# iyioon/NYPC-Yacht-Auction

Hardware: AMD Instinct MI355X
Metric: MCTS node-expansions/sec/GPU @4096 envs x100 sims; episodes/sec 1-8 GPU (higher is better)
Workload: dtype f32

## Files before the change

### nypc-yacht-auction_amd/csrc/yk_engine.hip

```cpp
#include <math.h>

#include <algorithm>
#include <vector>

#include "yk_api.h"
#include "yk_common.h"
#include "yk_engine_dev.h"
#include "yk_forced.h"
#include "yk_fpu.h"
#include "yk_net.h"

#define YK_MAX_GROUPS 8

using namespace yk;

namespace {


struct PwPlan {
    int nleaf, nop, root;
    uint16_t start[64], len[64];
    uint8_t a[64], b[64];
};
constexpr int pw_build(PwPlan& p, int start, int n) {
// ... 62 lines not shown
    int l = 0;
    for (int i = 0; i < p.nleaf; i++) l = p.len[i] > l ? p.len[i] : l;
    return l;
}
static_assert(NCOMB > pw_lmax(), "two category starts could share a leaf of the pairwise plan");
static_assert(PF_WCAP % 8 == 0 && PF_WCAP >= 16 && GAMES_PER_BLOCK * PF_WCAP * 4 <= 40 * 1024,
              "the prior window: whole float4 pairs, a slot per category, 16 waves per CU");
constexpr int PW_NLEAF = make_plan().nleaf;
constexpr int PW_SPLIT = make_plan().start[PW_NLEAF / 2];
static_assert(PW_SPLIT % 8 == 0 && PW_SPLIT <= PF_WCAP && ASIZE - PW_SPLIT <= PF_WCAP,
              "both halves of the pairwise tree fit the prior window, float4s aligned");
static_assert(PW_SPLIT > NBID && (PW_SPLIT - NBID) / NCOMB < NCAT, "the split lies inside a category's block");
constexpr int PW_SPLIT_CAT = (PW_SPLIT - NBID) / NCOMB, PW_SPLIT_COMB = (PW_SPLIT - NBID) % NCOMB;
constexpr int pw_leaf2() {
    const PwPlan p = make_plan();
    int i = 0;
    while (ASIZE - p.start[i] > PF_WCAP) i++;
    return i;
}
constexpr int PW_LEAF2 = pw_leaf2(), PW_BASE2 = make_plan().start[PW_LEAF2];
static_assert(PW_LEAF2 <= PW_NLEAF / 2 && PW_BASE2 % 8 == 0 && PW_BASE2 <= PW_SPLIT - (PW_SPLIT_COMB & 3),
              "the second piece holds the right half and the group the split cuts");

struct ValidQ {
    int mode;
    int n;
    uint32_t used;
    __device__ __forceinline__ bool operator()(int a) const {
        if (mode == 1) return a < NBID;
        if (mode != 0 || a < NBID) return false;
        const int base = a - NBID, cat = base / NCOMB, ci = base - cat * NCOMB;
        if ((used >> cat) & 1u) return false;
        if (n >= 10) return true;
        if (n == 5) return ci == 0;
        return c_tab.comb_max[ci] < n;
    }
};
__device__ __forceinline__ ValidQ valid_q(const YkS& s) {
    ValidQ q;
    const int round = s_round(s), phase = s_phase(s);
    const uint64_t wa = s_pw(s, 0, 0);
    q.n = __builtin_amdgcn_readfirstlane(wa_n(wa));
    q.used = __builtin_amdgcn_readfirstlane((uint32_t)wa_used(wa));
    q.mode = __builtin_amdgcn_readfirstlane((phase == 0 && round != 13) ? 1 : (phase == 1 && q.n >= 5) ? 0 : -1);
    return q;
}


__device__ __forceinline__ void wave_sync() {
    __builtin_amdgcn_fence(__ATOMIC_ACQ_REL, "workgroup");
    __builtin_amdgcn_wave_barrier();
}

__device__ __forceinline__ float wave_max(float v) {
    v = fmaxf(v, xlane<32>(v));
    v = fmaxf(v, xlane<16>(v));
    v = fmaxf(v, xlane<8>(v));
    v = fmaxf(v, xlane<4>(v));
    v = fmaxf(v, xlane<2>(v));
    return fmaxf(v, xlane<1>(v));
}
__device__ __forceinline__ float softmax_p(float x, float m, float lse) { return exp_acc(x - m - lse); }
__device__ __forceinline__ float wave_sumf(float v) {
    v += xlane<32>(v);
    v += xlane<16>(v);
    v += xlane<8>(v);
    v += xlane<4>(v);
    v += xlane<2>(v);
    return v + xlane<1>(v);
}
__device__ __forceinline__ int wave_min_i(int v) {
    v = min(v, xlane<32>(v));
    v = min(v, xlane<16>(v));
    v = min(v, xlane<8>(v));
    v = min(v, xlane<4>(v));
    v = min(v, xlane<2>(v));
    return min(v, xlane<1>(v));
}

struct PyV {
    double v;
    uint32_t t;
};
__device__ __forceinline__ PyV pv_update(PyV q, uint32_t n, PyV v) {
    PyV prod, sum, out;
    if (q.t == T_F32) prod = PyV{(double)((float)n * (float)q.v), T_F32};
    else prod = PyV{(double)n * q.v, q.t};
    if (prod.t == T_F32 || v.t == T_F32) sum = PyV{(double)((float)prod.v + (float)v.v), T_F32};
    else if (prod.t == T_F64 || v.t == T_F64) sum = PyV{prod.v + v.v, T_F64};
    else sum = PyV{prod.v + v.v, T_INT};
    if (sum.t == T_F32) out = PyV{(double)((float)sum.v / (float)(n + 1)), T_F32};
    else out = PyV{sum.v / (double)(n + 1), T_F64};
    return out;
}

__global__ void k_lut(float* sq, float* sqe) {
    const int i = blockIdx.x * blockDim.x + threadIdx.x;
    if (i >= LUT_N) return;
    sq[i] = (float)sqrt((double)i);
    sqe[i] = (float)sqrt((double)i + 1e-8);
}

__global__ void k_reset(EngDev d, int start_games, uint32_t env_base) {
    const int e = blockIdx.x * blockDim.x + threadIdx.x;
    if (e >= d.E) return;
    for (int t = e; t < d.T; t += d.E) {
        d.node_count[t] = d.node_count[d.T + t] = 0;
        d.edge_count[t] = d.edge_count[d.T + t] = 0;
        d.arena_top[t] = 0;
        d.gen[t] = 0;
        d.cur_round[t] = 0;
        d.root_c[2 * t] = make_uint4(0, 0, 0, 0);
        d.root_c[2 * t + 1] = make_uint4(0, 0, RV_OFF, 0);
    }
#pragma unroll
    for (int k = 0; k < GST; k++) d.gstats[(long)e * GST + k] = 0;
    if (!start_games) return;
    d.env_id[e] = env_base + (uint32_t)e;
    Stream rs{d.seed, d.env_id[e], 0};
    YkS s;
#pragma unroll
    for (int k = 0; k < 8; k++) s.w[k] = 0;
    s.w[0] = 1ull | NO_BIDS;
    new_round_rolls(s, rs);
    st_state(d.board + e, s);
    d.cur[e] = 1;
    d.ctr[e] = rs.ctr;
    d.done[e] = 0;
    d.nmoves[e] = 0;
    d.rec_voff[(long)e * (d.M + 1)] = 0;
}

__global__ __launch_bounds__(256) void k_move_begin(EngDev d, int move, int external_root) {
    const int lane = threadIdx.x & 63;
    const int e = d.e_lo + blockIdx.x * GAMES_PER_BLOCK + (threadIdx.x >> 6);
    if (e >= d.e_hi) return;
    const int t = tree_of(d, e);
    if (lane == 0) {
        d.root_c[2 * t] = make_uint4(0, 0, 0, 0);
        d.root_c[2 * t + 1] = make_uint4(0, 0, RV_OFF, 0);
    }
    if (!external_root) {
        if (d.done[e]) return;
        const YkS b = ld_state(d.board + e);
        const YkS r = canonical(b, d.cur[e]);
        const bool idle = d.arena && (d.cur[e] == d.seat[e] ? d.arena_agent : d.arena_opp) != YK_PLAYER_MCTS;
        if (lane == 0) {
            st_state(d.root + e, r);
            d.rec_ctr[((long)e * d.M + move) * 2] = d.ctr[e];
            d.idle[e] = idle ? 1 : 0;
        }
        if (idle) return;
    } else if (lane == 0) {
        d.idle[e] = 0;
    }
    const YkS r = ld_state(d.root + e);
    const int rr = s_round(r);
    const int cr = d.cur_round[t];
    if (rr == cr) return;
    if (rr < cr) {
        if (lane == 0) atomicOr(d.err, ERR_ROUND);
        return;
    }
    const int g = d.gen[t], h = g ^ 1;
    uint32_t* hx = d.hidx[h] + (long)t * d.HCAP;
    for (int i = lane; i < d.HCAP; i += 64) hx[i] = 0;
    const NodeRec* src = d.nodes[g] + (long)t * d.NCAP;
    NodeRec* dst = d.nodes[h] + (long)t * d.NCAP;
    const Edge* esrc = d.edges[g] + (long)t * d.ECAP;
// ... 126 lines not shown
        gathered += (uint64_t)nv;
        return -1;
    }
    if (FPU) {
        const int mine = bj;
        wave_argmax_step(best, bj);
        const uint64_t own = __ballot(mine == bj);
        wtag = own ? __builtin_amdgcn_readlane(btag, (int)__builtin_ctzll(own)) : 0u;
        const bool vis = bj != 0x7FFFFFFF;
        if (found && vis) {
            const float fq = fpu_value((int64_t)fpu_wave_sum((uint64_t)fw), fpu_wave_sum(fm), Ns, fr);
            fcnt = 1;
            if (fpu_unvisited_wins(fq, ub, uj, best, bj)) {
                fcnt = 3;
                best = ub;
                bj = uj;
                wtag = 0u;
            }
        } else if (found) {
            best = ub;
            bj = uj;
            wtag = 0u;
        }
        if (FORCED) fpick = best == INFINITY;
        scanned += (uint64_t)nv + (uint64_t)walked;
        gathered += (uint64_t)nv;
        return bj;
    }
    if (lane == 0 && found && (ub > best || (ub == best && uj < bj))) {
        best = ub;
        bj = uj;
        btag = 0;
    }
    const int mine = bj;
    wave_argmax_step(best, bj);
    if (FORCED) fpick = best == INFINITY;
    const uint64_t own = __ballot(mine == bj);
    wtag = own ? __builtin_amdgcn_readlane(btag, (int)__builtin_ctzll(own)) : 0u;
    scanned += (uint64_t)nv + (uint64_t)walked;
    gathered += (uint64_t)nv;
    return bj;
}

__device__ __forceinline__ void select_none(const EngDev& d, int e, int lane) {
    if (lane == 0) {
        d.leaf_flag[e] = 0;
        d.path_len[e] = 0;
        d.end_node[e] = 0;
    }
}

template <bool FORCED, bool FPU>
__device__ __forceinline__ void select_game(const EngDev& d, int e, int lane, int t, int g, const uint32_t* env_ids,
                                            uint64_t* ctr_arr, const ForcedDev& fd, const FpuDev& fp) {
    int fpick = 0;
    int fcnt = 0;
    int fpu_n = 0, fpu_u = 0;
    YkS s = ld_state(d.root + e);
    Stream rs{d.seed, env_ids[e], ctr_arr[e]};
    const NodeRec* nodes = d.nodes[g] + (long)t * d.NCAP;
    const Edge* edges = d.edges[g] + (long)t * d.ECAP;
    const float* Pbase = d.arenaP + (long)t * d.AE;
    const uint16_t* Sbase = d.arenaS + (long)t * d.AE;
    uint64_t* path = d.path + (long)e * MAXD;
    int depth = 0;
    uint64_t scanned = 0, gathered = 0;
    int ngl = 0;
    int leaf = 0;
    uint32_t end_id = 0;
    PyV res{0.0, T_INT};
    bool have = false;
    int nid = -1;
    NodeF f{};
    bool pre = false;
    int pre_bj = 0x7FFFFFFF;
    uint32_t pre_tag = 0;
    {
        const uint4 rc = d.root_c[2 * t], rc1 = d.root_c[2 * t + 1];
        const uint32_t rid = uni(rc.x);
        if (rid != 0) {
            have = true;
            nid = (int)rid - 1;
            f = ld_node(nodes + nid);
            f.p_off = rc.y;
            f.nvalid = rc.z;
            f.vinfo = (uint64_t)rc1.x | ((uint64_t)rc1.y << 32);
            f = uniform(f);
        }
        if (rid != 0 && uni(rc1.z) != RV_OFF) {
            const float sq = (float)sqrt((double)f.Ns), sqe = (float)sqrt((double)f.Ns + 1e-8);
            pre_bj = __builtin_amdgcn_readfirstlane(root_scan<FORCED, FPU>(
                d, t, lane, rc1.z, Pbase + rc.y, Sbase + rc.y, edges, (int)rc.z, (int)rc.w, (int)rc1.w, sq, sqe, pre_tag,
                scanned, gathered, f.Ns, fd.k, fpick, fp.r_root, fcnt));
            pre_tag = __builtin_amdgcn_readfirstlane(pre_tag);
            pre = pre_bj != -1;
            if (FORCED) fpick = pre ? __builtin_amdgcn_readfirstlane(fpick) : 0;
            if (FPU && pre) {
                fcnt = __builtin_amdgcn_readfirstlane(fcnt);
                fpu_n += fcnt & 1;
                fpu_u += fcnt >> 1;
            }
        }
    }
    while (true) {
        if (!have) {
            const double es = game_ended(s, 1);
            if (es != 0.0) {
                res = PyV{-es, T_F64};
                break;
            }
            const uint64_t hsh = index_hash(s);
            nid = __builtin_amdgcn_readfirstlane(lookup(d, g, t, s, hsh, f));
            f = uniform(f);
            if (nid < 0) {
                leaf = 1;
                if (lane == 0) {
                    st_state(d.leaf_state + e, s);
                    d.leaf_hash[e] = hsh;
                }
                break;
            }
            if (depth == 0 && lane == 0) {
                d.root_c[2 * t] = make_uint4((uint32_t)nid + 1, f.p_off, f.nvalid, 0);
                d.root_c[2 * t + 1] = make_uint4((uint32_t)f.vinfo, (uint32_t)(f.vinfo >> 32), RV_OFF, 0);
            }
        }
        const uint32_t p_off = f.p_off;
        const int V = (int)f.nvalid;
        const uint64_t vinfo = f.vinfo;
        if (V == 0) {
            res = PyV{0.0, T_INT};
            end_id = (uint32_t)nid + 1;
            break;
        }
        const uint32_t Ns = f.Ns;
        const float sq = (float)sqrt((double)Ns);
        const float sqe = (float)sqrt((double)Ns + 1e-8);
        const float* P = Pbase + p_off;
        const uint16_t* S = Sbase + p_off;
        int bj_out;
        uint32_t wtag;
        if (depth == 0 && pre) {
            bj_out = pre_bj;
            wtag = pre_tag;
        } else {
            float best = -INFINITY;
            int bj = 0x7FFFFFFF;
            uint32_t btag = 0;
            float bestx = -INFINITY;
            int bjx = 0x7FFFFFFF;
            int64_t fw = 0;
            uint64_t fm = 0;
            int Vs = V;
            if (d.node_summary && Ns == 0) {
                bj = (int)f.first_j;
                Vs = 0;
            }
            float4 p4 = make_float4(0.f, 0.f, 0.f, 0.f);
            ushort4 s4 = make_ushort4(0, 0, 0, 0);
            if (lane * 4 < Vs) {
                p4 = *reinterpret_cast<const float4*>(P + lane * 4);
                s4 = *reinterpret_cast<const ushort4*>(S + lane * 4);
            }
            for (int j0 = lane * 4; j0 < Vs; j0 += 256) {
                const float pv[4] = {p4.x, p4.y, p4.z, p4.w};
                const uint16_t sv[4] = {s4.x, s4.y, s4.z, s4.w};
                Edge ev[4];
#pragma unroll
                for (int t = 0; t < 4; t++)
                    if (j0 + t < Vs && sv[t]) {
                        ev[t] = edges[sv[t] - 1];
                        ngl++;
                    }
                if (j0 + 256 < Vs) {
                    p4 = *reinterpret_cast<const float4*>(P + j0 + 256);
                    s4 = *reinterpret_cast<const ushort4*>(S + j0 + 256);
                }
#pragma unroll
                for (int t = 0; t < 4; t++) {
                    const int j = j0 + t;
                    if (j < Vs) {
                        float u;
                        const float cp = d.c32 * pv[t];
                        if (sv[t]) {
                            u = (float)ev[t].Q + (cp * sq) / (float)(ev[t].N + 1);
                            if (FORCED && depth == 0 && forced_edge(ev[t].N, pv[t], Ns, fd.k)) u = INFINITY;
                        } else {
                            u = cp * sqe;
                        }
                        if (FPU) {
                            if (sv[t]) {
                                fw += fpu_w_term(ev[t].N, ev[t].Q);
                                fm += fpu_m_term(pv[t]);
                                if (u > best) {
                                    best = u;
                                    bj = j;
                                    btag = ev[t].tag;
                                }
                            } else if (u > bestx) {
                                bestx = u;
                                bjx = j;
                            }
                        } else if (u > best) {
                            best = u;
                            bj = j;
                            btag = sv[t] ? ev[t].tag : 0u;
                        }
                    }
                }
            }
            if (Vs) wave_argmax_step(best, bj);
            if (FPU && Vs) {
                wave_argmax_step(bestx, bjx);
                const bool vis = bj != 0x7FFFFFFF, unv = bjx != 0x7FFFFFFF;
                bool unv_won = unv;
                if (vis && unv) {
                    const float fq = fpu_value((int64_t)fpu_wave_sum((uint64_t)fw), fpu_wave_sum(fm), Ns, depth == 0 ? fp.r_root : fp.r);
                    unv_won = fpu_unvisited_wins(fq, bestx, bjx, best, bj);
                    fpu_n++;
                    fpu_u += unv_won;
                }
                if (unv_won) {
                    best = bestx;
                    bj = bjx;
                    btag = 0u;
                }
            }
            if (FORCED && depth == 0) fpick = best == INFINITY;
            scanned += (uint64_t)Vs;
            bj_out = bj;
            wtag = __builtin_amdgcn_readlane(btag, __builtin_amdgcn_readfirstlane((bj & 255) >> 2));
        }
        const int bj = bj_out;
        int j = bj;
        if (j == 0x7FFFFFFF) j = 0;
        if (depth >= MAXD) {
            if (lane == 0) atomicOr(d.err, ERR_DEPTH);
            res = PyV{0.0, T_INT};
            break;
        }
        const uint32_t child = uni(bj == 0x7FFFFFFF ? 0u : (wtag >> 2));
        if (child) {
            if (lane == 0) path[depth] = ((uint64_t)(p_off + (uint32_t)j) << 32) | (uint32_t)nid | PATH_DET;
            depth++;
            have = true;
            nid = (int)child - 1;
            f = uniform(ld_node(nodes + nid));
            s = ld_state(reinterpret_cast<const yk_state_t*>(nodes[nid].key));
            continue;
        }
        have = false;
        const VInfo vi = unpack_vinfo(vinfo, (uint32_t)V);
        const int a = compact_to_action(vi, j);
        int np = 1;
        const uint64_t ctr0 = rs.ctr;
        const int st = step_state<true>(s, 1, a, rs, np);
        const uint32_t det = rs.ctr == ctr0 ? PATH_DET : 0u;
        if (lane == 0) path[depth] = ((uint64_t)(p_off + (uint32_t)j) << 32) | (uint32_t)nid | det;
        depth++;
        if (st != YK_ST_OK) {
            if (lane == 0) atomicOr(d.err, ERR_STEP);
            res = PyV{0.0, T_INT};
            break;
        }
        s = canonical(s, np);
    }
    gathered += (uint64_t)xlane_sum(ngl);
    if (lane == 0) {
        d.leaf_flag[e] = (uint8_t)(leaf ? (t < d.E ? 1 : 2) : 0);
        d.path_len[e] = (uint8_t)depth;
        d.end_node[e] = end_id;
        d.res_v[e] = res.v;
        d.res_t[e] = res.t;
        ctr_arr[e] = rs.ctr;
        unsigned long long* gs = reinterpret_cast<unsigned long long*>(d.gstats + (long)e * GST);
        atomicAdd(gs + 1, (unsigned long long)scanned);
        atomicAdd(gs + 2, (unsigned long long)depth);
        atomicAdd(gs + 7, 1ull);
        if (FORCED) atomicAdd(gs + 12, (unsigned long long)fpick);
        if (FPU) {
            atomicAdd(gs + 14, (unsigned long long)fpu_u);
            atomicAdd(gs + 15, (unsigned long long)fpu_n);
        }
        atomicAdd(gs + 8, (unsigned long long)gathered);
    }
}

__device__ __forceinline__ ForcedDev forced_arg() { return ForcedDev{0.0, 0.0}; }
__device__ __forceinline__ const ForcedDev& forced_arg(const ForcedDev& fd) { return fd; }
__device__ __forceinline__ ForcedDev forced_arg(const FpuDev&) { return ForcedDev{0.0, 0.0}; }
__device__ __forceinline__ const ForcedDev& forced_arg(const ForcedDev& fd, const FpuDev&) { return fd; }
__device__ __forceinline__ FpuDev fpu_arg() { return FpuDev{0.0, 0.0}; }
__device__ __forceinline__ FpuDev fpu_arg(const ForcedDev&) { return FpuDev{0.0, 0.0}; }
__device__ __forceinline__ const FpuDev& fpu_arg(const FpuDev& fp) { return fp; }
__device__ __forceinline__ const FpuDev& fpu_arg(const ForcedDev&, const FpuDev& fp) { return fp; }
template <bool FORCED, bool FPU, class... FD>
__global__ __launch_bounds__(256) __attribute__((amdgpu_waves_per_eu(4))) void k_select(EngDev d, const uint32_t* env_ids, uint64_t* ctr_arr, FD... fd) {
    static_assert(sizeof...(FD) == (FORCED ? 1 : 0) + (FPU ? 1 : 0), "ForcedDev with FORCED, FpuDev with FPU, no further argument");
    const int lane = threadIdx.x & 63;
    const int e = __builtin_amdgcn_readfirstlane(d.e_lo + blockIdx.x * GAMES_PER_BLOCK + (threadIdx.x >> 6));
    if (e >= d.e_hi) return;
    if (d.done[e] || d.idle[e]) {
        select_none(d, e, lane);
        return;
    }
    const int t = __builtin_amdgcn_readfirstlane(tree_of(d, e));
    const int g = __builtin_amdgcn_readfirstlane((int)d.gen[t]);
    select_game<FORCED, FPU>(d, e, lane, t, g, env_ids, ctr_arr, forced_arg(fd...), fpu_arg(fd...));
}

__device__ __forceinline__ void expand_backup_game(const EngDev& d, int e, int lane, int t, int g);
template <bool FORCED, bool FPU, class... FD>
__global__ __launch_bounds__(256) __attribute__((amdgpu_waves_per_eu(YK_EXPAND_WPE))) void k_expand_backup(
    EngDev d, int do_select, const uint32_t* env_ids, uint64_t* ctr_arr, FD... fd) {
    static_assert(sizeof...(FD) == (FORCED ? 1 : 0) + (FPU ? 1 : 0), "ForcedDev with FORCED, FpuDev with FPU, no further argument");
    const int lane = threadIdx.x & 63;
    const int e = __builtin_amdgcn_readfirstlane(d.e_lo + blockIdx.x * GAMES_PER_BLOCK + (threadIdx.x >> 6));
    if (e >= d.e_hi) return;
    if (d.done[e]) return;
    const int t = __builtin_amdgcn_readfirstlane(tree_of(d, e));
    const int g = __builtin_amdgcn_readfirstlane((int)d.gen[t]);
    const bool idle = d.idle[e] != 0;
    expand_backup_game(d, e, lane, t, g);
    if (do_select) {
        if (idle) {
            select_none(d, e, lane);
            return;
        }
        wave_sync();
        select_game<FORCED, FPU>(d, e, lane, t, g, env_ids, ctr_arr, forced_arg(fd...), fpu_arg(fd...));
    }
}

__device__ __forceinline__ void expand_backup_game(const EngDev& d, int e, int lane, int t, int g) {
    PyV res{d.res_v[e], d.res_t[e]};
    uint32_t end_id = 0;
    if (d.leaf_flag[e]) {
        const YkS s = ld_state(d.leaf_state + e);
        const uint64_t ihsh = d.leaf_hash[e];
        const uint64_t hsh = d.prior == 1 ? key_hash(s) : 0ull;
        const VInfo vi = valid_info(s, 1);
        const ValidQ valid = valid_q(s);
        const int V = vi.V;
        const int leaf = lane >> 1, h = lane & 1;
        const int st = c_pw.start[leaf], nl = c_pw.len[leaf], G = nl >> 3, R = nl & 7;
        float4 q[PW_GMAX];
        float qt[PW_TMAX];
        float v, mx = 0.f, lse = 0.f;
        const int pidx = (int)d.gstats[(long)e * GST + 0];
        const bool rec = d.rec_pred && (e % d.rec_stride) == 0 && pidx < d.max_exp;
        const long rslot = rec ? (long)(e / d.rec_stride) * d.max_exp + pidx : 0;
        bool masked = false;
        __shared__ __attribute__((aligned(16))) float s_win[GAMES_PER_BLOCK][PF_WCAP];
        float* win = s_win[threadIdx.x >> 6];
        int fast = 0, wbase = 0, wlen = 0;
        if (d.prior_fast && V > 0) {
            if (valid.mode == 0 && valid.n == 5) {
                fast = 2;
                wlen = 16;
            } else {
                const int a0 = __builtin_amdgcn_readfirstlane(compact_to_action(vi, 0));
                const int a1 = __builtin_amdgcn_readfirstlane(compact_to_action(vi, V - 1));
                wbase = a0 & ~7;
                wlen = (a1 + 1 - wbase + 7) & ~7;
                fast = wlen <= PF_WCAP ? 1 : 0;
            }
        }
        const auto wslot = [&](int a) { return fast == 2 ? (a - NBID) / NCOMB : a - wbase; };
        if (d.prior == 0) {
            const float2 ml = d.mlse[e];
            mx = ml.x;
            lse = ml.y;
            if (d.fparts > 1) {
                float ms = ml.y;
                for (int p = 1; p < d.fparts; p++) {
                    const float2 q = d.mlse[(long)p * d.E + e];
                    const float mm = fmaxf(mx, q.x);
                    if (mm != -INFINITY) {
                        ms = ms * exp_acc(mx - mm) + q.y * exp_acc(q.x - mm);
                        mx = mm;
                    }
                }
                lse = logf(ms);
            }
            v = d.vpred[e];
        } else {
            v = hash_prior_v(hsh);
        }
        if (fast) {
            for (int i = 4 * lane; i < wlen; i += 256) *reinterpret_cast<float4*>(win + i) = make_float4(0.f, 0.f, 0.f, 0.f);
            wave_sync();
            const float* __restrict__ xr = d.logits + (long)e * PI_LD;
            for (int j0 = lane; j0 < V; j0 += 256) {
                float xa[4];
                int aa[4];
#pragma unroll
                for (int u = 0; u < 4; u++) {
                    const int j = j0 + 64 * u;
                    aa[u] = j < V ? compact_to_action(vi, j) : 0;
                    xa[u] = (d.prior == 0 && j < V) ? xr[aa[u]] : 0.f;
                }
#pragma unroll
                for (int u = 0; u < 4; u++)
                    if (j0 + 64 * u < V)
                        win[wslot(aa[u])] = d.prior == 0 ? softmax_p(xa[u], mx, lse) : hash_prior_pi(hsh, aa[u]);
            }
            wave_sync();
// ... 965 lines not shown
        }
    }
    const size_t R = ((size_t)cfg->n_envs + d.rec_stride - 1) / d.rec_stride;
    const size_t E = (size_t)d.E, T = (size_t)d.T;
#define A(p, n) YK_TRY(eng->mem.alloc(&(p), (n)))
    for (int g = 0; g < 2; g++) {
        A(d.nodes[g], T * d.NCAP);
        A(d.hidx[g], T * d.HCAP);
        A(d.edges[g], T * d.ECAP);
    }
    A(d.node_count, 2 * T);
    A(d.edge_count, 2 * T);
    A(d.arenaP, T * (size_t)d.AE);
    A(d.arenaS, T * (size_t)d.AE);
    A(d.arena_top, T);
    A(d.gen, T);
    A(d.cur_round, T);
    A(d.root_c, 2 * T);
    A(d.rv, T * RV_CAP);
    A(d.ro_j, T * RO_K);
    A(d.ro_p, T * RO_K);
    A(d.board, E);
    A(d.cur, E);
    A(d.ctr, E);
    A(d.env_id, E);
    A(d.done, E);
    A(d.nmoves, E);
    A(d.root, E);
    A(d.leaf_state, E);
    A(d.leaf_hash, E);
    A(d.leaf_flag, E);
    A(d.path, E * MAXD);
    A(d.path_len, E);
    A(d.end_node, E);
    A(d.res_v, E);
    A(d.res_t, E);
    A(eng->vpred, E);
    A(eng->mlse, E * (size_t)d.fparts);
    A(eng->lut_sq, (size_t)LUT_N);
    A(eng->lut_sqe, (size_t)LUT_N);
    A(d.rec_state, E * d.M);
    A(d.rec_info, E * d.M * 8);
    A(d.rec_ctr, E * d.M * 2);
    A(d.rec_val, E * d.M);
    A(d.rec_visits, E * (size_t)d.VCAP);
    A(d.rec_voff, E * (d.M + 1));
    A(d.final_r, E);
    A(d.final_cur, E);
    A(d.final_tot, 2 * E);
    A(d.seat, E);
    A(d.idle, E);
    A(d.gstats, E * GST);
    A(d.err, 1);
    A(eng->done_count, 1);
    A(eng->mcts_env, E);
    if (d.prior == 0) {
        A(eng->logits, E * (size_t)PI_LD);
    }
    eng->root_values = cfg->record_root_values != 0;
    eng->noise = cfg->dirichlet_alpha > 0.0 && cfg->dirichlet_eps > 0.0;
    eng->nz.alpha = cfg->dirichlet_alpha;
    eng->nz.eps = cfg->dirichlet_eps;
    if (eng->noise) {
        A(eng->nz.noised, E);
        if (d.rec_pred) {
            A(eng->nz.prior_before, R * (size_t)d.M * ASIZE);
            A(eng->nz.prior_after, R * (size_t)d.M * ASIZE);
        }
    }
    if (d.rec_pred) {
        A(d.rec_pi, R * (size_t)d.max_exp * ASIZE);
        A(d.rec_v, R * (size_t)d.max_exp);
        A(d.rec_leaf, R * (size_t)d.max_exp);
    }
#undef A
    if (hipHostMalloc((void**)&eng->host_done, sizeof(int32_t)) != hipSuccess) return YK_ERR_NOMEM;
    {
        const char* ev = getenv("YK_ROOT_SCAN");
        eng->root_scan = !(ev && ev[0] == '0');
        const char* ek = getenv("YK_ROOT_K");
        d.ro_k = ek ? std::max(1, std::min(RO_K, atoi(ek))) : RO_K;
        const char* en = getenv("YK_NODE_SUMMARY");
        d.node_summary = (en && en[0] == '0') ? 0 : 1;
        const char* ep = getenv("YK_PRIOR_FAST");
        d.prior_fast = !ep ? 2 : (ep[0] == '0' && !ep[1]) ? 0 : (ep[0] == '1' && !ep[1]) ? 1 : 2;
        const char* es = getenv("YK_SPLIT_DESCENT");
        eng->split_descent = es && es[0] == '1';
    }
    if (G > 1) {
        if (hipEventCreateWithFlags(&eng->ev_fork, hipEventDisableTiming) != hipSuccess) return YK_ERR_HIP;
        for (int g = 0; g < G; g++)
            if (hipStreamCreateWithFlags(&eng->gs[g], hipStreamNonBlocking) != hipSuccess ||
                hipEventCreateWithFlags(&eng->ev_join[g], hipEventDisableTiming) != hipSuccess ||
                hipEventCreateWithFlags(&eng->ev_fwd[g], hipEventDisableTiming) != hipSuccess)
                return YK_ERR_HIP;
    }
    if (eng->fparts_dual > 0) {
        if (hipStreamCreateWithFlags(&eng->dstream, hipStreamNonBlocking) != hipSuccess ||
            hipEventCreateWithFlags(&eng->ev_d0, hipEventDisableTiming) != hipSuccess ||
            hipEventCreateWithFlags(&eng->ev_d1, hipEventDisableTiming) != hipSuccess)
            return YK_ERR_HIP;
    }
    d.logits = eng->logits;
    d.vpred = eng->vpred;
    d.mlse = eng->mlse;
    d.lut_sq = eng->lut_sq;
    d.lut_sqe = eng->lut_sqe;
    hipLaunchKernelGGL(k_lut, dim3(LUT_N / 256), dim3(256), 0, 0, eng->lut_sq, eng->lut_sqe);
    YK_LAUNCHED();
    YK_HIP(hipMemset(d.err, 0, sizeof(uint32_t)));
    YK_HIP(hipMemset(d.done, 0, E));
    YK_HIP(hipMemset(d.idle, 0, E));
    YK_HIP(hipMemset(d.leaf_state, 0, sizeof(yk_state_t) * E));
    std::vector<uint32_t> ids(E);
    for (size_t i = 0; i < E; i++) ids[i] = (uint32_t)i;
    YK_HIP(hipMemcpy(eng->mcts_env, ids.data(), sizeof(uint32_t) * E, hipMemcpyHostToDevice));
    YK_HIP(hipDeviceSynchronize());
    *out = eng.release();
    return YK_OK;
}

int yk_engine_destroy(yk_engine_t* eng) {
    delete eng;
    return YK_OK;
}

}

namespace {
bool playout_full(uint64_t seed, uint32_t env_base, int move, double full_prob) {
    return u53(philox_u64(philox4x32_10(seed, (uint32_t)move, env_base, 0u, PHILOX_PLAYOUT))) < full_prob;
}

int play_batch(yk_engine* eng, uint64_t seed, uint32_t env_base, hipStream_t s) {
    EngDev& d = eng->d;
    d.seed = seed;
    const int G = eng->ngroups;
    hipStream_t st[YK_MAX_GROUPS];
    EngDev dg[YK_MAX_GROUPS];
    for (int g = 0; g < G; g++) {
        st[g] = G == 1 ? s : eng->gs[g];
        dg[g] = G == 1 ? d : group_dev(eng, g);
    }
    const dim3 bb(256);
    YK_HIP(hipMemsetAsync(d.err, 0, sizeof(uint32_t), s));
    YK_HIP(hipMemsetAsync(d.hidx[0], 0, sizeof(uint32_t) * (size_t)d.T * d.HCAP, s));
    const bool noise = eng->noise && !d.arena;
    const bool root_values = eng->root_values && !d.arena;
    const bool capped = eng->fast_sims > 0 && !d.arena;
    eng->have_priors = false;
    eng->fast_moves = 0;
    const bool forcing = eng->forced_k > 0.0 && !d.arena;
    const ForcedDev fd{eng->forced_k, eng->cfg.cpuct};
    if (root_values)
        YK_HIP(hipMemsetAsync(d.rec_info, 0, sizeof(int32_t) * (size_t)d.E * d.M * 8, s));
    if (noise && eng->nz.prior_after) {
        const size_t nb = sizeof(float) * (((size_t)d.E + d.rec_stride - 1) / d.rec_stride) * (size_t)d.M * ASIZE;
        YK_HIP(hipMemsetAsync(eng->nz.prior_before, 0, nb, s));
        YK_HIP(hipMemsetAsync(eng->nz.prior_after, 0, nb, s));
    }
    hipLaunchKernelGGL(k_reset, dim3((d.E + 255) / 256), dim3(256), 0, s, d, 1, env_base);
    YK_LAUNCHED();
    if (G > 1) {
// ... 160 lines not shown
        eng->klaunch[i] = 0;
    }
    return YK_OK;
}

int yk_engine_kernel_times(yk_engine_t* eng, double* ms, int64_t* launches) {
    if (!eng || !ms || !launches) return YK_ERR_ARG;
    for (int i = 0; i < 8; i++) {
        ms[i] = eng->kms[i];
        launches[i] = eng->klaunch[i];
    }
    return YK_OK;
}

int yk_engine_stats(yk_engine_t* eng, int64_t* out) {
    if (!eng || !out) return YK_ERR_ARG;
    EngDev& d = eng->d;
    std::vector<uint64_t> gs((size_t)d.E * GST);
    std::vector<int32_t> nm(d.E);
    uint32_t err = 0;
    YK_HIP(hipDeviceSynchronize());
    YK_HIP(hipMemcpy(gs.data(), d.gstats, sizeof(uint64_t) * gs.size(), hipMemcpyDeviceToHost));
    YK_HIP(hipMemcpy(nm.data(), d.nmoves, sizeof(int32_t) * nm.size(), hipMemcpyDeviceToHost));
    YK_HIP(hipMemcpy(&err, d.err, sizeof(uint32_t), hipMemcpyDeviceToHost));
    for (int i = 0; i < 16; i++) out[i] = 0;
    for (int e = 0; e < d.E; e++) {
        const uint64_t* g = &gs[(size_t)e * GST];
        out[0] += (int64_t)g[0];
        out[1] += (int64_t)g[1];
        out[2] = std::max<int64_t>(out[2], nm[e]);
        out[4] = std::max<int64_t>(out[4], (int64_t)g[4]);
        out[5] = std::max<int64_t>(out[5], (int64_t)g[5]);
        out[6] = std::max<int64_t>(out[6], (int64_t)g[6]);
        out[7] += (int64_t)g[3];
        out[8] += (int64_t)g[2];
        out[9] = std::max<int64_t>(out[9], (int64_t)g[7]);
    }
    out[3] = err;
    out[10] = d.NCAP;
    out[11] = d.ECAP;
    out[12] = d.AE;
    out[13] = d.VCAP;
    out[14] = eng->ngroups;
    out[15] = d.fparts;
    return YK_OK;
}

int yk_engine_counters(yk_engine_t* eng, int64_t* out, int n) {
    if (!eng || !out || n < 0) return YK_ERR_ARG;
    EngDev& d = eng->d;
    std::vector<uint64_t> gs((size_t)d.E * GST);
    YK_HIP(hipDeviceSynchronize());
    YK_HIP(hipMemcpy(gs.data(), d.gstats, sizeof(uint64_t) * gs.size(), hipMemcpyDeviceToHost));
    int64_t c[9] = {0, 0, 0, 0, eng->fast_moves, 0, 0, 0, 0};
    for (int e = 0; e < d.E; e++) {
        c[0] += (int64_t)gs[(size_t)e * GST + 8];
        for (int k = 0; k < 3; k++) c[1 + k] += (int64_t)gs[(size_t)e * GST + 9 + k];
        for (int k = 0; k < 4; k++) c[5 + k] += (int64_t)gs[(size_t)e * GST + 12 + k];
    }
    for (int i = 0; i < n; i++) out[i] = i < 9 ? c[i] : 0;
    return YK_OK;
}

int yk_engine_records(yk_engine_t* eng, uint64_t* states, int32_t* info, uint64_t* ctr, double* values,
                      uint64_t* final_states, int32_t* n_moves, int64_t* visits_off, int32_t* visits,
                      int64_t* n_visits) {
    if (!eng) return YK_ERR_ARG;
    if (!eng->have_records) return YK_ERR_STATE;
    EngDev& d = eng->d;
    const size_t E = d.E, M = d.M;
    YK_HIP(hipDeviceSynchronize());
    if (states) YK_HIP(hipMemcpy(states, d.rec_state, sizeof(yk_state_t) * E * M, hipMemcpyDeviceToHost));
    if (info) YK_HIP(hipMemcpy(info, d.rec_info, sizeof(int32_t) * E * M * 8, hipMemcpyDeviceToHost));
    if (ctr) YK_HIP(hipMemcpy(ctr, d.rec_ctr, sizeof(uint64_t) * E * M * 2, hipMemcpyDeviceToHost));
    if (values) YK_HIP(hipMemcpy(values, d.rec_val, sizeof(double) * E * M, hipMemcpyDeviceToHost));
    if (final_states) YK_HIP(hipMemcpy(final_states, d.board, sizeof(yk_state_t) * E, hipMemcpyDeviceToHost));
    if (n_moves) YK_HIP(hipMemcpy(n_moves, d.nmoves, sizeof(int32_t) * E, hipMemcpyDeviceToHost));
    if (visits_off || visits || n_visits) {
        std::vector<int32_t> voff(E * (M + 1));
        std::vector<int32_t> nm(E);
        YK_HIP(hipMemcpy(voff.data(), d.rec_voff, sizeof(int32_t) * voff.size(), hipMemcpyDeviceToHost));
        YK_HIP(hipMemcpy(nm.data(), d.nmoves, sizeof(int32_t) * E, hipMemcpyDeviceToHost));
        int64_t total = 0;
        for (size_t e = 0; e < E; e++) total += voff[e * (M + 1) + nm[e]];
        if (n_visits) *n_visits = total;
        if (visits_off || visits) {
            std::vector<uint32_t> raw(E * (size_t)d.VCAP);
            YK_HIP(hipMemcpy(raw.data(), d.rec_visits, sizeof(uint32_t) * raw.size(), hipMemcpyDeviceToHost));
            int64_t k = 0;
            for (size_t e = 0; e < E; e++) {
                for (size_t m = 0; m < M; m++) {
                    const int32_t a0 = voff[e * (M + 1) + m];
                    const int32_t a1 = (int)m < nm[e] ? voff[e * (M + 1) + m + 1] : a0;
                    if (visits_off) visits_off[e * M + m] = k;
                    for (int32_t i = a0; i < a1; i++, k++)
                        if (visits) {
                            const uint32_t x = raw[e * d.VCAP + i];
                            visits[2 * k] = (int32_t)(x >> 16);
                            visits[2 * k + 1] = (int32_t)(x & 0xFFFF);
                        }
                }
            }
            if (visits_off) visits_off[E * M] = k;
        }
    }
    return YK_OK;
}

int yk_engine_predictions(yk_engine_t* eng, float* pi, float* v, yk_state_t* leaves, int32_t* count) {
    if (!eng || !eng->d.rec_pred) return YK_ERR_ARG;
    EngDev& d = eng->d;
    const size_t R = ((size_t)d.E + d.rec_stride - 1) / d.rec_stride, X = (size_t)d.max_exp;
    YK_HIP(hipDeviceSynchronize());
// ... 102 lines not shown
```

### nypc-yacht-auction_amd/csrc/yk_engine_dev.h

```cpp
#pragma once
#include <math.h>
#include <stddef.h>

#include <type_traits>

#include "yk_api.h"
#include "yk_common.h"

using namespace yk;

namespace {

constexpr int MAXD = 64;
constexpr int LUT_N = 1 << 16;
constexpr int GAMES_PER_BLOCK = 4;
constexpr int GROUP_ALIGN = 16;
constexpr int YK_EXPAND_WPE = 4;
constexpr int RO_CAP = 3072;
constexpr int RO_K = 512;
constexpr int RV_CAP = 1024;
constexpr uint32_t RV_OFF = 0xFFFFFFFFu;
constexpr int PF_WCAP = 2048;

enum : uint32_t { T_INT = 0, T_F64 = 1, T_F32 = 2 };

struct NodeRec {
    uint64_t key[8];
    uint64_t hash;
    uint64_t vinfo;
    uint32_t p_off;
    uint32_t nvalid;
    uint32_t Ns;
    uint32_t first_j;
};
static_assert(sizeof(NodeRec) == 96, "NodeRec: 96 bytes");
struct Edge {
    double Q;
    uint32_t N;
    uint32_t tag;
};
__device__ __forceinline__ uint32_t edge_kind(uint32_t tag) { return tag & 3u; }
constexpr uint32_t PATH_DET = 0x80000000u;

constexpr int GST = 16;
struct EngDev {
    int E, NCAP, HCAP, ECAP, M, VCAP;
    int e_lo, e_hi;
    int T, dual;
    int64_t AE;
    int sims, temp_threshold;
    float c32;
    int prior;
    int fparts;
    int rec_pred, max_exp, rec_stride;
    int arena;
    int arena_agent, arena_opp;
    uint64_t seed;
    NodeRec* nodes[2];
    uint32_t* hidx[2];
    Edge* edges[2];
    uint32_t* node_count;
    uint32_t* edge_count;
    float* arenaP;
    uint16_t* arenaS;
    uint32_t* arena_top;
    uint8_t* gen;
    uint8_t* cur_round;
    uint4* root_c;
    int node_summary;
    int prior_fast;
    int ro_k;
    uint32_t* rv;
    uint16_t* ro_j;
    float* ro_p;
    yk_state_t* board;
    int32_t* cur;
    uint64_t* ctr;
    uint32_t* env_id;
    uint8_t* done;
    int32_t* nmoves;
    yk_state_t* root;
    int32_t* seat;
    uint8_t* idle;
    yk_state_t* leaf_state;
    uint64_t* leaf_hash;
    uint8_t* leaf_flag;
    uint64_t* path;
    uint8_t* path_len;
    uint32_t* end_node;
    double* res_v;
    uint32_t* res_t;
    const float* logits;
    const float* vpred;
    const float2* mlse;
    const float* lut_sq;
    const float* lut_sqe;
    yk_state_t* rec_state;
    int32_t* rec_info;
    uint64_t* rec_ctr;
    double* rec_val;
    uint32_t* rec_visits;
    int32_t* rec_voff;
    double* final_r;
    int32_t* final_cur;
    int32_t* final_tot;
    float* rec_pi;
    float* rec_v;
    yk_state_t* rec_leaf;
    uint64_t* gstats;
    uint32_t* err;
};

struct NoiseDev {
    double alpha, eps;
    uint8_t* noised;
    float* prior_before;
    float* prior_after;
};

struct RootValDev {
    int move;
};

enum : uint32_t {
// ... 124 lines not shown
```

### nypc-yacht-auction_amd/yacht_amd/engine.py

```python
from __future__ import annotations

import ctypes as C

import numpy as np
import torch

from ._lib import YK_REC_FAST, YkEngineConfigFull, call, lib, stream_ptr

ACTION_SIZE = 3226


class SelfPlayEngine:
    def __init__(self, n_envs: int, sims: int, cpuct: float = 1.5, temp_threshold: int = 15, net=None,
                 prior: str = "net", max_moves: int = 64, record_predictions: bool = False,
                 max_expansions: int = 0, arena_entries: int = 0, record_stride: int = 1, groups: int = 0,
                 dual_trees: bool = False, opponent_net=None, dirichlet_alpha: float = 0.0,
                 dirichlet_eps: float = 0.0, record_root_values: bool = False, playout_fast_sims: int = 0,
                 playout_full_prob: float = 1.0, forced_playouts_k: float = 0.0, forced_prune: bool = True,
                 fpu_reduction=None, fpu_root_reduction=None):
        if prior not in ("net", "hash"):
            raise ValueError("prior is 'net' (YachtNNet on MFMA) or 'hash' (deterministic test prior)")
        if prior == "net" and net is None:
            raise ValueError("prior='net' needs a YkNet")
        self.cfg = YkEngineConfigFull(
# ... 49 lines not shown
        try:
            call("yk_selfplay", self.handle, seed & (2**64 - 1), env_base & (2**32 - 1), stream_ptr(stream))
        except YkError as e:
            st = self.stats()
            bits = [n for b, n in self.ERROR_BITS.items() if st["errors"] & b]
            raise YkError(f"yk_selfplay [{', '.join(bits)}; stats {st}]", e.code) from None

    PLAYERS = {"mcts": 0, "random": 1, "greedy": 2}

    def arena(self, agent_seat, seed: int, env_base: int = 0, stream=None, agent: str = "mcts",
              opponent: str = "random"):
        from ._lib import YkError
        seat = np.ascontiguousarray(np.broadcast_to(np.asarray(agent_seat, dtype=np.int32), (self.n_envs,)))
        try:
            call("yk_arena", self.handle, seed & (2**64 - 1), env_base & (2**32 - 1), seat.ctypes.data,
                 self.PLAYERS[agent], self.PLAYERS[opponent], stream_ptr(stream))
        except YkError as e:
            st = self.stats()
            bits = [n for b, n in self.ERROR_BITS.items() if st["errors"] & b]
            raise YkError(f"yk_arena [{', '.join(bits)}; stats {st}]", e.code) from None

    def arena_results(self) -> dict:
        E, M = self.n_envs, self.max_moves
        result = np.zeros(E, dtype=np.float64)
        totals = np.zeros((E, 2), dtype=np.int32)
        nm = np.zeros(E, dtype=np.int32)
        actions = np.zeros((E, M), dtype=np.int32)
        final = np.zeros((E, 8), dtype=np.uint64)
        ctr = np.zeros(E, dtype=np.uint64)
        call("yk_arena_results", self.handle, result.ctypes.data, totals.ctypes.data, nm.ctypes.data,
             actions.ctypes.data, final.ctypes.data, ctr.ctypes.data)
        return dict(result=result, totals=totals, n_moves=nm, actions=actions, final=final, ctr=ctr)

    KERNEL_CLASSES = ("select", "forward", "root_sort_select", "expand_backup_select", "move_begin", "move_end")

    def profile(self, enable: bool = True, stride: int = 1):
        call("yk_engine_profile", self.handle, int(stride) if enable else 0)

    def kernel_times(self) -> dict:
        ms = np.zeros(8, dtype=np.float64)
        n = np.zeros(8, dtype=np.int64)
        call("yk_engine_kernel_times", self.handle, ms.ctypes.data, n.ctypes.data)
        kt = {k: (float(ms[i]), int(n[i])) for i, k in enumerate(self.KERNEL_CLASSES) if k != "unused"}
        if self.cfg.dirichlet_alpha > 0 and self.cfg.dirichlet_eps > 0:
            kt["root_noise"] = (float(ms[6]), int(n[6]))
        if self.cfg.record_root_values:
            kt["root_value"] = (float(ms[7]), int(n[7]))
        return kt

    STAT_NAMES = ("expansions", "scanned", "moves", "errors", "max_nodes", "max_edges", "max_arena", "vnew",
                  "path_edges", "sims", "node_cap", "edge_cap", "arena_cap", "visit_cap", "groups",
                  "forward_parts")
    COUNTER_NAMES = ("scan_edges", "prior_window", "prior_sparse", "prior_general", "fast_moves", "forced_picks",
                     "pruned_visits", "fpu_unvisited_picks", "fpu_picks")

    def stats(self) -> dict:
        out = np.zeros(16, dtype=np.int64)
        call("yk_engine_stats", self.handle, out.ctypes.data)
        st = {k: int(out[i]) for i, k in enumerate(self.STAT_NAMES)}
        more = np.zeros(len(self.COUNTER_NAMES), dtype=np.int64)
        if hasattr(lib(), "yk_engine_counters"):
            call("yk_engine_counters", self.handle, more.ctypes.data, len(more))
        st.update({k: int(more[i]) for i, k in enumerate(self.COUNTER_NAMES)})
        return st

    def records(self) -> dict:
        E, M = self.n_envs, self.max_moves
        states = np.zeros((E, M, 8), dtype=np.uint64)
        info = np.zeros((E, M, 8), dtype=np.int32)
        ctr = np.zeros((E, M, 2), dtype=np.uint64)
        values = np.zeros((E, M), dtype=np.float64)
        final = np.zeros((E, 8), dtype=np.uint64)
        nm = np.zeros(E, dtype=np.int32)
        nv = np.zeros(1, dtype=np.int64)
        call("yk_engine_records", self.handle, None, None, None, None, None, None, None, None, nv.ctypes.data)
        voff = np.zeros(E * M + 1, dtype=np.int64)
        visits = np.zeros((max(int(nv[0]), 1), 2), dtype=np.int32)
        call("yk_engine_records", self.handle, states.ctypes.data, info.ctypes.data, ctr.ctypes.data,
             values.ctypes.data, final.ctypes.data, nm.ctypes.data, voff.ctypes.data, visits.ctypes.data,
             nv.ctypes.data)
        rec = dict(states=states, info=info, ctr=ctr, values=values, final=final, n_moves=nm,
                   visits_off=voff.reshape(-1)[:E * M + 1], visits=visits[:int(nv[0])])
        if self.cfg.record_root_values:
            rec["root_values"] = decode_root_values(info[:, :, 7])
        if self.playout_fast_sims > 0:
            rec["fast"] = ((info[:, :, 6] & YK_REC_FAST) != 0) & (np.arange(M)[None, :] < nm[:, None])
        return rec

    def predictions(self, leaves: bool = False):
        R = (self.n_envs + self.cfg.record_stride - 1) // self.cfg.record_stride
        X = self.cfg.max_expansions
        pi = np.zeros((R, X, ACTION_SIZE), dtype=np.float32)
        v = np.zeros((R, X), dtype=np.float32)
        lv = np.zeros((R, X, 8), dtype=np.uint64) if leaves else None
        cnt = np.zeros(R, dtype=np.int32)
        call("yk_engine_predictions", self.handle, pi.ctypes.data, v.ctypes.data,
             lv.ctypes.data if leaves else None, cnt.ctypes.data)
        if (cnt > X).any():
            raise RuntimeError(f"prediction record truncated: {int(cnt.max())} expansions > max_expansions {X}")
        return (pi, v, cnt, lv) if leaves else (pi, v, cnt)

    def root_priors(self):
        R = (self.n_envs + self.cfg.record_stride - 1) // self.cfg.record_stride
        before = np.zeros((R, self.max_moves, ACTION_SIZE), dtype=np.float32)
        after = np.zeros_like(before)
        call("yk_engine_root_priors", self.handle, before.ctypes.data, after.ctypes.data)
        return before, after
# ... 52 lines not shown
```

Measured before the change: 33.01 million.

## Split wide PUCT child scans into unvisited-only pass plus compacted visited gather

For nodes with many children (above a runtime threshold), the selection scan now runs in two phases. First it streams priors and slot indices with a multi-stage prefetch and scores unvisited children from the prior alone. Visited children are compacted into a shared-memory list via ballot/mbcnt, then gathered densely in a second pass, flushing when the list fills. The goal is to avoid scattered edge loads for mostly-unvisited wide nodes, at the cost of extra shared memory, wave syncs and a global atomic flush counter.

Result: no change. 33.25 million (median of 6 runs) (+0.7%).

```diff
diff --git a/nypc-yacht-auction_amd/csrc/yk_engine.hip b/nypc-yacht-auction_amd/csrc/yk_engine.hip
--- a/nypc-yacht-auction_amd/csrc/yk_engine.hip
+++ b/nypc-yacht-auction_amd/csrc/yk_engine.hip
@@ -138,6 +138,15 @@
     __builtin_amdgcn_wave_barrier();
 }
 
+__device__ __forceinline__ uint32_t lanes_below(uint64_t bal) {
+    return __builtin_amdgcn_mbcnt_hi((uint32_t)(bal >> 32), __builtin_amdgcn_mbcnt_lo((uint32_t)bal, 0u));
+}
+#ifndef YK_SCAN_DEPTH
+#define YK_SCAN_DEPTH 3
+#endif
+static_assert(YK_SCAN_DEPTH >= 1 && YK_SCAN_DEPTH <= 4, "the scan's stage: one to four iterations");
+constexpr int scan_depth(bool forced, bool fpu) { return (forced && fpu && YK_SCAN_DEPTH > 2) ? 2 : YK_SCAN_DEPTH; }
+
 __device__ __forceinline__ float wave_max(float v) {
     v = fmaxf(v, xlane<32>(v));
     v = fmaxf(v, xlane<16>(v));
@@ -201,6 +210,7 @@
     }
 #pragma unroll
     for (int k = 0; k < GST; k++) d.gstats[(long)e * GST + k] = 0;
+    if (e == 0) *d.scan_flushes = 0;
     if (!start_games) return;
     d.env_id[e] = env_base + (uint32_t)e;
     Stream rs{d.seed, d.env_id[e], 0};
@@ -433,7 +443,7 @@
 
 template <bool FORCED, bool FPU>
 __device__ __forceinline__ void select_game(const EngDev& d, int e, int lane, int t, int g, const uint32_t* env_ids,
-                                            uint64_t* ctr_arr, const ForcedDev& fd, const FpuDev& fp) {
+                                            uint64_t* ctr_arr, const ForcedDev& fd, const FpuDev& fp, uint32_t* lst) {
     int fpick = 0;
     int fcnt = 0;
     int fpu_n = 0, fpu_u = 0;
@@ -537,13 +547,100 @@
                 bj = (int)f.first_j;
                 Vs = 0;
             }
+            const bool split = d.scan_split && Vs >= d.scan_split;
+            if (split) {
+                constexpr int SD = scan_depth(FORCED, FPU);
+                const int Vu = __builtin_amdgcn_readfirstlane(Vs);
+                float4 pq[SD];
+                ushort4 sq4[SD];
+#pragma unroll
+                for (int k = 0; k < SD; k++) {
+                    pq[k] = make_float4(0.f, 0.f, 0.f, 0.f);
+                    sq4[k] = make_ushort4(0, 0, 0, 0);
+                    if (k * 256 + lane * 4 < Vu) {
+                        pq[k] = *reinterpret_cast<const float4*>(P + (uint32_t)(k * 256 + lane * 4));
+                        sq4[k] = *reinterpret_cast<const ushort4*>(S + (uint32_t)(k * 256 + lane * 4));
+                    }
+                }
+                int jb = 0, nl = 0;
+                do {
+                    while (jb < Vu && nl < d.scan_cap) {
+#pragma unroll
+                        for (int k = 0; k < SD; k++) {
+                            if (jb < Vu) {
+                                const int j0 = jb + lane * 4;
+                                const float pv[4] = {pq[k].x, pq[k].y, pq[k].z, pq[k].w};
+                                const uint16_t sv[4] = {sq4[k].x, sq4[k].y, sq4[k].z, sq4[k].w};
+                                bool anyv = false;
+#pragma unroll
+                                for (int t = 0; t < 4; t++) {
+                                    const int j = j0 + t;
+                                    const float u = (d.c32 * pv[t]) * sqe;
+                                    const bool in = j < Vu;
+                                    const bool tk = in & (sv[t] == 0) & (u > bestx);
+                                    bestx = tk ? u : bestx;
+                                    bjx = tk ? j : bjx;
+                                    anyv |= in & (sv[t] != 0);
+                                }
+                                if (__ballot(anyv)) {
+#pragma unroll
+                                    for (int t = 0; t < 4; t++) {
+                                        const bool vis = j0 + t < Vu && sv[t];
+                                        const uint64_t bal = __ballot(vis);
+                                        if (vis) lst[nl + (int)lanes_below(bal)] = (uint32_t)(j0 + t) | ((uint32_t)sv[t] << 12);
+                                        nl += __popcll(bal);
+                                    }
+                                }
+                                if (j0 + SD * 256 < Vu) {
+                                    pq[k] = *reinterpret_cast<const float4*>(P + (uint32_t)(j0 + SD * 256));
+                                    sq4[k] = *reinterpret_cast<const ushort4*>(S + (uint32_t)(j0 + SD * 256));
+                                }
+                                jb += 256;
+                            }
+                        }
+                    }
+                    if (nl) {
+                        wave_sync();
+                        for (int i = lane; i < nl; i += 64) {
+                            const uint32_t w = lst[i];
+                            const int j = (int)(w & 0xFFFu);
+                            const Edge ev = edges[(w >> 12) - 1];
+                            const float p = P[w & 0xFFFu];
+                            const float cp = d.c32 * p;
+                            float u = (float)ev.Q + (cp * sq) / (float)(ev.N + 1);
+                            if (FORCED && depth == 0 && forced_edge(ev.N, p, Ns, fd.k)) u = INFINITY;
+                            if (FPU) {
+                                fw += fpu_w_term(ev.N, ev.Q);
+                                fm += fpu_m_term(p);
+                            }
+                            if (u > best || (u == best && j < bj && u != -INFINITY)) {
+                                best = u;
+                                bj = j;
+                                btag = ev.tag;
+                            }
+                        }
+                        gathered += (uint64_t)nl;
+                        nl = 0;
+                        if (jb < Vu) {
+                            if (lane == 0) atomicAdd(d.scan_flushes, 1u);
+                            wave_sync();
+                        }
+                    }
+                } while (jb < Vu);
+                if (!FPU && (bestx > best || (bestx == best && bjx < bj))) {
+                    best = bestx;
+                    bj = bjx;
+                    btag = 0u;
+                }
+            }
+            const int Vo = split ? 0 : Vs;
             float4 p4 = make_float4(0.f, 0.f, 0.f, 0.f);
             ushort4 s4 = make_ushort4(0, 0, 0, 0);
-            if (lane * 4 < Vs) {
+            if (lane * 4 < Vo) {
                 p4 = *reinterpret_cast<const float4*>(P + lane * 4);
                 s4 = *reinterpret_cast<const ushort4*>(S + lane * 4);
             }
-            for (int j0 = lane * 4; j0 < Vs; j0 += 256) {
+            for (int j0 = lane * 4; j0 < Vo; j0 += 256) {
                 const float pv[4] = {p4.x, p4.y, p4.z, p4.w};
                 const uint16_t sv[4] = {s4.x, s4.y, s4.z, s4.w};
                 Edge ev[4];
@@ -590,7 +687,9 @@
                     }
                 }
             }
+            const int mine = bj;
             if (Vs) wave_argmax_step(best, bj);
+            const int wl = (int)__builtin_ctzll(__ballot(mine == bj));
             if (FPU && Vs) {
                 wave_argmax_step(bestx, bjx);
                 const bool vis = bj != 0x7FFFFFFF, unv = bjx != 0x7FFFFFFF;
@@ -610,7 +709,7 @@
             if (FORCED && depth == 0) fpick = best == INFINITY;
             scanned += (uint64_t)Vs;
             bj_out = bj;
-            wtag = __builtin_amdgcn_readlane(btag, __builtin_amdgcn_readfirstlane((bj & 255) >> 2));
+            wtag = __builtin_amdgcn_readlane(btag, split ? wl : __builtin_amdgcn_readfirstlane((bj & 255) >> 2));
         }
         const int bj = bj_out;
         int j = bj;
@@ -687,10 +786,11 @@
     }
     const int t = __builtin_amdgcn_readfirstlane(tree_of(d, e));
     const int g = __builtin_amdgcn_readfirstlane((int)d.gen[t]);
-    select_game<FORCED, FPU>(d, e, lane, t, g, env_ids, ctr_arr, forced_arg(fd...), fpu_arg(fd...));
-}
-
-__device__ __forceinline__ void expand_backup_game(const EngDev& d, int e, int lane, int t, int g);
+    __shared__ uint32_t s_lst[GAMES_PER_BLOCK][PF_WCAP];
+    select_game<FORCED, FPU>(d, e, lane, t, g, env_ids, ctr_arr, forced_arg(fd...), fpu_arg(fd...), s_lst[threadIdx.x >> 6]);
+}
+
+__device__ __forceinline__ void expand_backup_game(const EngDev& d, int e, int lane, int t, int g, float* win);
 template <bool FORCED, bool FPU, class... FD>
 __global__ __launch_bounds__(256) __attribute__((amdgpu_waves_per_eu(YK_EXPAND_WPE))) void k_expand_backup(
     EngDev d, int do_select, const uint32_t* env_ids, uint64_t* ctr_arr, FD... fd) {
@@ -702,18 +802,21 @@
     const int t = __builtin_amdgcn_readfirstlane(tree_of(d, e));
     const int g = __builtin_amdgcn_readfirstlane((int)d.gen[t]);
     const bool idle = d.idle[e] != 0;
-    expand_backup_game(d, e, lane, t, g);
+    __shared__ __attribute__((aligned(16))) float s_win[GAMES_PER_BLOCK][PF_WCAP];
+    float* win = s_win[threadIdx.x >> 6];
+    expand_backup_game(d, e, lane, t, g, win);
     if (do_select) {
         if (idle) {
             select_none(d, e, lane);
             return;
         }
         wave_sync();
-        select_game<FORCED, FPU>(d, e, lane, t, g, env_ids, ctr_arr, forced_arg(fd...), fpu_arg(fd...));
-    }
-}
-
-__device__ __forceinline__ void expand_backup_game(const EngDev& d, int e, int lane, int t, int g) {
+        select_game<FORCED, FPU>(d, e, lane, t, g, env_ids, ctr_arr, forced_arg(fd...), fpu_arg(fd...),
+                                 reinterpret_cast<uint32_t*>(win));
+    }
+}
+
+__device__ __forceinline__ void expand_backup_game(const EngDev& d, int e, int lane, int t, int g, float* win) {
     PyV res{d.res_v[e], d.res_t[e]};
     uint32_t end_id = 0;
     if (d.leaf_flag[e]) {
@@ -732,8 +835,6 @@
         const bool rec = d.rec_pred && (e % d.rec_stride) == 0 && pidx < d.max_exp;
         const long rslot = rec ? (long)(e / d.rec_stride) * d.max_exp + pidx : 0;
         bool masked = false;
-        __shared__ __attribute__((aligned(16))) float s_win[GAMES_PER_BLOCK][PF_WCAP];
-        float* win = s_win[threadIdx.x >> 6];
         int fast = 0, wbase = 0, wlen = 0;
         if (d.prior_fast && V > 0) {
             if (valid.mode == 0 && valid.n == 5) {
@@ -1805,6 +1906,7 @@
     A(d.idle, E);
     A(d.gstats, E * GST);
     A(d.err, 1);
+    A(d.scan_flushes, 1);
     A(eng->done_count, 1);
     A(eng->mcts_env, E);
     if (d.prior == 0) {
@@ -1837,6 +1939,10 @@
         d.node_summary = (en && en[0] == '0') ? 0 : 1;
         const char* ep = getenv("YK_PRIOR_FAST");
         d.prior_fast = !ep ? 2 : (ep[0] == '0' && !ep[1]) ? 0 : (ep[0] == '1' && !ep[1]) ? 1 : 2;
+        const char* ess = getenv("YK_SCAN_SPLIT");
+        d.scan_split = ess ? std::max(0, std::min(RO_CAP + 1, atoi(ess))) : SCAN_SPLIT_MIN;
+        const char* ec = getenv("YK_SCAN_LIST_CAP");
+        d.scan_cap = ec ? std::max(1, std::min(SCAN_LIST_CAP, atoi(ec))) : SCAN_LIST_CAP;
         const char* es = getenv("YK_SPLIT_DESCENT");
         eng->split_descent = es && es[0] == '1';
     }
@@ -1862,6 +1968,7 @@
     hipLaunchKernelGGL(k_lut, dim3(LUT_N / 256), dim3(256), 0, 0, eng->lut_sq, eng->lut_sqe);
     YK_LAUNCHED();
     YK_HIP(hipMemset(d.err, 0, sizeof(uint32_t)));
+    YK_HIP(hipMemset(d.scan_flushes, 0, sizeof(uint32_t)));
     YK_HIP(hipMemset(d.done, 0, E));
     YK_HIP(hipMemset(d.idle, 0, E));
     YK_HIP(hipMemset(d.leaf_state, 0, sizeof(yk_state_t) * E));
@@ -2128,13 +2235,15 @@
     std::vector<uint64_t> gs((size_t)d.E * GST);
     YK_HIP(hipDeviceSynchronize());
     YK_HIP(hipMemcpy(gs.data(), d.gstats, sizeof(uint64_t) * gs.size(), hipMemcpyDeviceToHost));
-    int64_t c[9] = {0, 0, 0, 0, eng->fast_moves, 0, 0, 0, 0};
+    uint32_t fl = 0;
+    YK_HIP(hipMemcpy(&fl, d.scan_flushes, sizeof(uint32_t), hipMemcpyDeviceToHost));
+    int64_t c[10] = {0, 0, 0, 0, eng->fast_moves, 0, 0, 0, 0, (int64_t)fl};
     for (int e = 0; e < d.E; e++) {
         c[0] += (int64_t)gs[(size_t)e * GST + 8];
         for (int k = 0; k < 3; k++) c[1 + k] += (int64_t)gs[(size_t)e * GST + 9 + k];
         for (int k = 0; k < 4; k++) c[5 + k] += (int64_t)gs[(size_t)e * GST + 12 + k];
     }
-    for (int i = 0; i < n; i++) out[i] = i < 9 ? c[i] : 0;
+    for (int i = 0; i < n; i++) out[i] = i < 10 ? c[i] : 0;
     return YK_OK;
 }
 
diff --git a/nypc-yacht-auction_amd/csrc/yk_engine_dev.h b/nypc-yacht-auction_amd/csrc/yk_engine_dev.h
--- a/nypc-yacht-auction_amd/csrc/yk_engine_dev.h
+++ b/nypc-yacht-auction_amd/csrc/yk_engine_dev.h
@@ -21,6 +21,8 @@
 constexpr int RV_CAP = 1024;
 constexpr uint32_t RV_OFF = 0xFFFFFFFFu;
 constexpr int PF_WCAP = 2048;
+constexpr int SCAN_LIST_CAP = PF_WCAP - 4 * 256;
+constexpr int SCAN_SPLIT_MIN = 512;
 
 enum : uint32_t { T_INT = 0, T_F64 = 1, T_F32 = 2 };
 
@@ -70,6 +72,9 @@
     int node_summary;
     int prior_fast;
     int ro_k;
+    int scan_split;
+    int scan_cap;
+    uint32_t* scan_flushes;
     uint32_t* rv;
     uint16_t* ro_j;
     float* ro_p;
diff --git a/nypc-yacht-auction_amd/yacht_amd/engine.py b/nypc-yacht-auction_amd/yacht_amd/engine.py
--- a/nypc-yacht-auction_amd/yacht_amd/engine.py
+++ b/nypc-yacht-auction_amd/yacht_amd/engine.py
@@ -125,7 +125,7 @@
                   "path_edges", "sims", "node_cap", "edge_cap", "arena_cap", "visit_cap", "groups",
                   "forward_parts")
     COUNTER_NAMES = ("scan_edges", "prior_window", "prior_sparse", "prior_general", "fast_moves", "forced_picks",
-                     "pruned_visits", "fpu_unvisited_picks", "fpu_picks")
+                     "pruned_visits", "fpu_unvisited_picks", "fpu_picks", "scan_flushes")
 
     def stats(self) -> dict:
         out = np.zeros(16, dtype=np.int64)
```
